# lzhangbj/DualVar

Measured on AMD Instinct MI355X. Metric: clips/sec (whole node), S3D-G 8x112^2 SimCLR pretrain step, higher is better.
Workload: dtype fp32

## Files before the change

dualvar_amd/csrc/conv.hip:

```cpp
#include "conv_common.hpp"

int dvt_conv_tap_kind(const void* conv_args, int mode);
int dvt_conv_tap_rows(const void* conv_args, int mode);
int dvt_conv_tap_launch(const void* conv_args, int mode, void* stream);
int64_t dvt_bn_ws_floats(int64_t rows, int np);
int dvt_conv_pp_rows(const void* conv_args, int mode);
int dvt_conv_pp_launch(const void* conv_args, int mode, void* stream);
void dvx_dgrad_bn_tail_launch(const void* conv_args, int is_f32, void* stream);

namespace {

constexpr int conv_waves_per_simd(int es, int gvb, int bm, int bn) {
  return (es == 4 && gvb == 16 && bm == 256) ? 3 : (es != 2 || gvb != 16) ? 1 : (bm * bn == 128 * 64) ? 6 : (bm == 128 && bn == 128) ? 3 : 1;
}

template <typename T, int MODE, int GVB, int BM, int BN, int WAVES_M, int WAVES_N, int GM, int NS = 2, bool SPLIT = false,
          bool WF = false, bool BNL = false>
__global__ __launch_bounds__(WAVES_M * WAVES_N * 64)
__attribute__((amdgpu_waves_per_eu(conv_waves_per_simd(sizeof(T), GVB, BM, BN)))) void conv_gemm_kernel(ConvArgs a) {
  static_assert(!SPLIT || sizeof(T) == 4, "the bf16 split is the fp32 mode's product");
  static_assert(!WF || (SPLIT && GVB == 16), "pre-split weights belong to the fp32 split kernels");
  static_assert(!BNL || (WF && GM == 1 && MODE == MODE_FWD), "BatchNorm on load: forward, uniform-tap gathers, pre-split weights");
  constexpr bool DMA = (GVB == 16);
  static_assert(GM == 0 || DMA, "uniform-tap gathers are DMA only");
// ... 1954 lines not shown
    p.BI = 64; p.BJ = (tmk == 3 ? 3 : d->kt) * bc;
    p.nti = (d->Cout + 63) / 64; p.ntj = (d->cin_pitch + bc - 1) / bc;
    const int krows = tmk == 3 ? 3 : 1;
    if (tmk == 4) {
      p.BJ = 224; p.ntj = 1;
      p.nchunks = d->N * d->To * d->Ho;
    } else if (tmk == 3) {
      p.nchunks = (M + 63) / 64;
    } else {
      const int pxs = 64 / d->To;
      p.nchunks = (int)(((int64_t)d->N * d->Hi * d->Wi + pxs - 1) / pxs);
    }
    int splits = std::max(1, ((tmk == 2 || tmk == 4) ? 512 : 768) / (p.nti * p.ntj * krows));
    splits = std::min(splits, std::max(1, p.nchunks / 8));
    const double slab_us = 8.0 * d->Cout * (double)J / 4e6;
    const int s_opt = (int)(std::sqrt(p.nchunks * 1.2 / slab_us) + 0.5);
    splits = std::max(1, std::min(splits, s_opt));
    p.chunks_per_split = (p.nchunks + splits - 1) / splits;
    p.splits = (p.nchunks + p.chunks_per_split - 1) / p.chunks_per_split;
    p.rows_per_split = p.chunks_per_split * 64;
    p.slab_stride = ((long long)d->Cout * J + 63) / 64 * 64;
    return p;
  }
  static const int f32s_force = env_int("DUALVAR_WGRAD_F32S", -1);
  const int f32s_pick = (f32s_force == 0 || f32s_force == 2) ? f32s_force : -1;
  if (p.dma && d->dtype == DV_F32 && !f32_exact() && f32s_pick >= 0) {
    p.f32s = f32s_pick;
    dvx_wgrad_f32s_tile(f32s_pick, &p.BI, &p.BJ);
    per_cu = std::max(1, std::min(2, 163840 / dvx_wgrad_f32s_lds_bytes(f32s_pick)));
  } else if (p.dma) {
    const WgradCfg* tab = d->dtype == DV_F32 ? kWgF32 : kWgBf16;
    const int ncfg = d->dtype == DV_F32 ? 2 : 4;
    constexpr int minrows_ = 256;
    double best = 0;
    for (int c = 0; c < ncfg; ++c) {
      const WgradCfg& k = tab[c];
      const int nti = (d->Cout + k.BI - 1) / k.BI, ntj = (J + k.BJ - 1) / k.BJ;
      const double fill = (double)M * nti * ntj * (k.BI + k.BJ) * es / 18e12;
      const double mfma = 2.0 * M * (double)(nti * k.BI) * (ntj * k.BJ) / (d->dtype == DV_F32 ? 120e12 : 1600e12);
      const int cap = 256 * wgrad_wgs_per_cu(es, k.BI, k.BJ, k.WVI * k.WVJ, k.NS);
      const int64_t sp = std::max<int64_t>(1, std::min<int64_t>(cap / (nti * ntj), (M + minrows_ - 1) / minrows_));
      const double wgs = (double)nti * ntj * sp;
      const double t = std::max(fill, mfma) * std::max(1.0, 256.0 / wgs);
      if (p.cfg < 0 || t < best) { best = t; p.cfg = c; }
    }
    const WgradCfg& k = tab[p.cfg];
    p.BI = k.BI; p.BJ = k.BJ;
    per_cu = wgrad_wgs_per_cu(es, k.BI, k.BJ, k.WVI * k.WVJ, k.NS);
  } else {
    const bool narrow = (d->Cout + 63) / 64 * 64 < (d->Cout + 127) / 128 * 128;
    p.BI = narrow ? 64 : 128;
    p.BJ = narrow ? 128 : 64;
  }
  p.nti = (d->Cout + p.BI - 1) / p.BI;
  p.ntj = (J + p.BJ - 1) / p.BJ;
  const int tiles = p.nti * p.ntj;
  constexpr int minrows = 256;
  const int tgt = 256 * per_cu;
  int splits = tgt / tiles;
  const int max_splits = (M + minrows - 1) / minrows;
  if (splits > max_splits) splits = max_splits;
  {
    const double t_step = d->dtype == DV_F32 ? 1.5 : 0.7;
    const double slab_us = 8.0 * d->Cout * (double)J / 4e6;
    const int s_opt = (int)(std::sqrt(M / 32.0 * t_step / slab_us) + 0.5);
    if (splits > s_opt) splits = s_opt;
  }
  if (splits < 1) splits = 1;
  p.rows_per_split = ((M + splits - 1) / splits + 31) / 32 * 32;
  p.splits = (M + p.rows_per_split - 1) / p.rows_per_split;
  p.slab_stride = ((long long)d->Cout * J + 63) / 64 * 64;
  return p;
}

extern "C" int dv_conv3d_wgrad_tile(const dv_conv_desc* d, int32_t* rows, int32_t* cols, int32_t* splits) {
  if (!d || !rows || !cols || !splits) return DV_EINVAL;
  int rc = check_desc(d);
  if (rc) return rc;
  const WgradPlan p = plan_wgrad(d);
  *rows = p.BI; *cols = p.BJ; *splits = p.splits;
  return DV_OK;
}

extern "C" int64_t dv_conv3d_wgrad_workspace(const dv_conv_desc* d) {
  if (check_desc(d)) return 0;
  const WgradPlan p = plan_wgrad(d);
  return p.splits > 1 ? (int64_t)p.splits * p.slab_stride * 4 : 0;
}

static bool wgrad_plan_is_share(const dv_conv_desc* d, const WgradPlan& p) {
  if (p.tm) return wgrad_tm_kind(d) == 4;
  return p.dma && d->dtype == DV_F32 && !f32_exact() && p.f32s < 0 && p.cfg == 1;
}
extern "C" int dv_conv3d_wgrad_bn_ok(const dv_conv_desc* d) {
  if (!d || check_desc(d)) return 0;
  return wgrad_plan_is_share(d, plan_wgrad(d)) ? 1 : 0;
}

static int wgrad_impl(const dv_conv_desc* d, const void* x, const void* dy, float* dw, void* workspace,
                      int64_t workspace_bytes, const dv_bn_bwd* bn, void* stream, const dv_bn_in* bn_in = nullptr) {
  int rc = check_desc(d);
  if (rc) return rc;
  if (!x || !dy || !dw) return DV_EINVAL;
  if (!aligned16(dy) || !aligned16(dw) || (reinterpret_cast<uintptr_t>(x) & 7)) return DV_EALIGN;
  const WgradPlan p = plan_wgrad(d);
  if (bn_in) {
    if (bn || !bn_in->scale || !bn_in->shift) return DV_EINVAL;
    const int k = p.tm ? wgrad_tm_kind(d) : 0;
    if (k != 1 && k != 2) return DV_EUNSUPPORTED;
  }
  if (bn) {
    if (!bn->x || !bn->mean || !bn->invstd || !bn->gamma || !bn->sums || bn->n_rep <= 0) return DV_EINVAL;
    if ((bn->dgamma == nullptr) != (bn->dbeta == nullptr)) return DV_EINVAL;
    if (!(bn->flags & DV_NO_RELU_MASK) && (!bn->scale || !bn->shift)) return DV_EINVAL;
    if (bn->ldx != d->ldy) return DV_EINVAL;
    if (!aligned16(bn->x)) return DV_EALIGN;
    if (!wgrad_plan_is_share(d, p)) return DV_EUNSUPPORTED;
  }
  const int64_t need = p.splits > 1 ? (int64_t)p.splits * p.slab_stride * 4 : 0;
  if (need && (!workspace || workspace_bytes < need)) return DV_EINVAL;
  if (need && !aligned16(workspace)) return DV_EALIGN;
  if (p.gvb == 16 && !aligned16(x)) return DV_EALIGN;
  WgradArgs a;
  fill_geom(d, MODE_FWD, a.g);
  a.x = x; a.dy = dy; a.dw = dw;
  a.slab = need ? reinterpret_cast<float*>(workspace) : nullptr;
  a.slab_stride = p.slab_stride;
  a.M = d->N * d->To * d->Ho * d->Wo;
  a.Cout = d->Cout; a.CoutP = d->cout_pitch; a.J = a.g.Ktot;
  a.ldx = d->ldx; a.ldy = d->ldy; a.ldw = a.g.Ktot;
  a.nti = p.nti; a.ntj = p.ntj;
  a.rows_per_split = p.rows_per_split;
  a.perm = make_row_perm(d->kt > 1 && d->To > 1, d->To, d->Ho * d->Wo);
  const int grid = p.nti * p.ntj * p.splits;
  const bool narrow = p.BI == 64;
  hipStream_t s = (hipStream_t)stream;
  if (p.tm) {
    TmWgradArgs t;
    t.x = x; t.dy = dy; t.dw = dw; t.slab = a.slab; t.slab_stride = p.slab_stride;
    t.S = d->Hi * d->Wi; t.NQ = d->N * t.S; t.T = d->To; t.kind = wgrad_tm_kind(d);
    t.Cout = d->Cout; t.CoutP = d->cout_pitch; t.CP = d->cin_pitch;
    t.ldx = d->ldx; t.ldy = d->ldy; t.ldw = a.ldw;
    t.nti = p.nti; t.ntc = p.ntj; t.nchunks = p.nchunks; t.chunks_per_split = p.chunks_per_split;
    t.x_bytes = (int)(((int64_t)d->N * d->Ti * d->Hi * d->Wi - 1) * d->ldx * 4 + (int64_t)d->cin_pitch * 4);
    t.dy_bytes = (int)(((int64_t)a.M - 1) * d->ldy * 4 + (int64_t)d->cout_pitch * 4);
    t.fS = make_fastdiv((uint32_t)t.S);
    t.M = a.M; t.H = d->Hi; t.W = d->Wi;
    t.fW = make_fastdiv((uint32_t)d->Wi); t.fH = make_fastdiv((uint32_t)d->Hi);
    t.Wo = d->Wo; t.Ho = d->Ho; t.Wp = d->Wi; t.Hp = d->Hi;
    t.bn_x = nullptr;
    if (bn_in) { t.in_scale = bn_in->scale; t.in_shift = bn_in->shift; t.in_C = d->Cin; t.in_relu = (bn_in->flags & DV_RELU) ? 1 : 0; }
    if (t.kind == 4) {
      t.fH = make_fastdiv((uint32_t)d->Ho);
      if (bn) {
        t.bn_x = bn->x; t.bn_mean = bn->mean; t.bn_invstd = bn->invstd; t.bn_gamma = bn->gamma; t.bn_scale = bn->scale;
        t.bn_shift = bn->shift; t.bn_sums = bn->sums; t.bn_dgamma = bn->dgamma; t.bn_dbeta = bn->dbeta;
        t.bn_inv_count = bn->inv_count; t.bn_dscale = bn->dparam_scale; t.bn_rep = bn->n_rep;
        t.bn_mask = (bn->flags & DV_NO_RELU_MASK) ? 0 : 1;
      }
    }
    dvw_wgrad_tm_launch(&t, t.kind == 3 ? grid * 3 : grid, stream);
  } else if (p.dma) {
    const int64_t es = d->dtype == DV_F32 ? 4 : 2;
    WgradDmaArgs aa;
    aa.w = a;
    aa.x_bytes = (int)(((int64_t)d->N * d->Ti * d->Hi * d->Wi - 1) * d->ldx * es + (int64_t)d->cin_pitch * es);
    aa.dy_bytes = (int)(((int64_t)a.M - 1) * d->ldy * es + (int64_t)d->cout_pitch * es);
    aa.bn_x = nullptr;
    if (bn) {
      aa.bn_x = bn->x; aa.bn_mean = bn->mean; aa.bn_invstd = bn->invstd; aa.bn_gamma = bn->gamma; aa.bn_scale = bn->scale;
      aa.bn_shift = bn->shift; aa.bn_sums = bn->sums; aa.bn_dgamma = bn->dgamma; aa.bn_dbeta = bn->dbeta;
      aa.bn_inv_count = bn->inv_count; aa.bn_dscale = bn->dparam_scale; aa.bn_rep = bn->n_rep;
      aa.bn_mask = (bn->flags & DV_NO_RELU_MASK) ? 0 : 1;
    }
#define WGD(T_, BI_, BJ_, WI_, WJ_, NS_, ...) \
  hipLaunchKernelGGL((conv_wgrad_dma_kernel<T_, BI_, BJ_, WI_, WJ_, NS_, ##__VA_ARGS__>), dim3(grid), dim3(WI_ * WJ_ * 64), 0, s, aa)
    if (p.f32s >= 0) {
      dvx_launch_wgrad_f32s(p.f32s, &aa, grid, s);
    } else if (d->dtype == DV_BF16) {
      switch (p.cfg) {
        case 0: WGD(bf16_t, 128, 128, 2, 2, 3); break;
        case 1: WGD(bf16_t, 64, 256, 1, 4, 3); break;
        case 2: WGD(bf16_t, 128, 256, 2, 2, 3); break;
        default: WGD(bf16_t, 192, 256, 3, 4, 4); break;
      }
    } else {
      if (f32_exact()) {
        if (p.cfg == 1) WGD(float, 64, 128, 2, 2, 2);
        else WGD(float, 128, 128, 2, 2, 2);
      } else {
        if (bn) WGD(float, 64, 128, 1, 4, 2, true, true, true);
        else if (p.cfg == 1) WGD(float, 64, 128, 1, 4, 2, true, true);
        else WGD(float, 128, 128, 2, 2, 2, true);
      }
    }
#undef WGD
  } else {
#define WG_LAUNCH(T_, G_)                                                                                   \
  do {                                                                                                      \
    if (narrow) hipLaunchKernelGGL((conv_wgrad_kernel<T_, G_, 64, 128>), dim3(grid), dim3(256), 0, s, a);   \
    else hipLaunchKernelGGL((conv_wgrad_kernel<T_, G_, 128, 64>), dim3(grid), dim3(256), 0, s, a);          \
  } while (0)
    if (d->dtype == DV_F32) WG_LAUNCH(float, 16);
    else if (p.gvb == 16) WG_LAUNCH(bf16_t, 16);
    else WG_LAUNCH(bf16_t, 8);
#undef WG_LAUNCH
  }
  if (need) {
    const long long n4 = (long long)d->Cout * a.ldw / 4;
    hipLaunchKernelGGL(wgrad_reduce_kernel, dim3((unsigned)((n4 + 15) / 16)), dim3(256), 0, s, a.slab, p.slab_stride,
                       p.splits, dw, n4);
  }
  return dv_launch_status();
}

extern "C" int dv_conv3d_wgrad(const dv_conv_desc* d, const void* x, const void* dy, float* dw, void* workspace,
                               int64_t workspace_bytes, void* stream) {
  return wgrad_impl(d, x, dy, dw, workspace, workspace_bytes, nullptr, stream);
}

extern "C" int dv_conv3d_wgrad_bn(const dv_conv_desc* d, const void* x, const void* g, float* dw, void* workspace,
                                  int64_t workspace_bytes, const dv_bn_bwd* bn, void* stream) {
  if (!bn) return DV_EINVAL;
  return wgrad_impl(d, x, g, dw, workspace, workspace_bytes, bn, stream);
}

extern "C" int dv_conv3d_wgrad_bn_in(const dv_conv_desc* d, const void* x_bn, const dv_bn_in* bn, const void* dy, float* dw,
                                     void* workspace, int64_t workspace_bytes, void* stream) {
  if (!bn) return DV_EINVAL;
  return wgrad_impl(d, x_bn, dy, dw, workspace, workspace_bytes, nullptr, stream, bn);
}

extern "C" int dv_conv3d_bn_in_ok(const dv_conv_desc* d) {
  if (!d || check_desc(d)) return 0;
  const int k = wgrad_tm_kind(d);
  if (k != 1 && k != 2) return 0;
  return fwd_bn_in_path(d);
}
```

dualvar_amd/csrc/conv_common.hpp:

```cpp
#pragma once
#include "common.hpp"
#include <algorithm>
#include <cmath>
#include <cstdlib>
#include <type_traits>
#include <utility>


namespace {


enum { MODE_FWD = 0, MODE_DGRAD = 1 };

struct ConvGeom {
  int rT, rH, rW;
  int sT, sH, sW;
  int kt, kh, kw;
  int st, sh, sw;
  int pt, ph, pw;
  int CP;
  int Ktot;
  FastDiv dW, dH, dT;
};

// ... 192 lines not shown
};
template <> struct Mma<fp8e5_t> {
  static __device__ __forceinline__ void tile(const unsigned char* a_row, const unsigned char* b_row, int h, int sa, int sb, f32x16& acc) {
    mma_fp8<1, 0>(a_row, b_row, h, sa, sb, acc);
  }
};
template <typename T> struct OutOf { typedef T type; };
template <> struct OutOf<fp8e4_t> { typedef bf16_t type; };
template <> struct OutOf<fp8e5_t> { typedef bf16_t type; };

struct Split3 { bf16x8 hi, mid, lo; };
__device__ __forceinline__ Split3 split3(const float (&v)[8]) {
  Split3 s;
#pragma unroll
  for (int e = 0; e < 8; ++e) {
    const bf16_t h = (bf16_t)v[e];
    const float r1 = v[e] - (float)h;
    const bf16_t m = (bf16_t)r1;
    const float r2 = r1 - (float)m;
    s.hi[e] = h; s.mid[e] = m; s.lo[e] = (bf16_t)r2;
  }
  return s;
}
__device__ __forceinline__ void split3w_pair(float x0, float x1, unsigned& H, unsigned& Mi, unsigned& Lo) {
  typedef __attribute__((ext_vector_type(2))) float f32x2;
  typedef __attribute__((ext_vector_type(2))) unsigned u32x2;
  typedef __attribute__((ext_vector_type(2))) __bf16 bf16x2;
  const u32x2 mask = {0xffff0000u, 0xffff0000u};
  const f32x2 x = {x0, x1};
  const bf16x2 hb = __builtin_convertvector(x, bf16x2);
  const unsigned hw = __builtin_bit_cast(unsigned, hb);
  const u32x2 hwide = {hw << 16, hw & 0xffff0000u};
  const f32x2 r1 = x - __builtin_bit_cast(f32x2, hwide);
  const u32x2 rb = __builtin_bit_cast(u32x2, r1);
  const f32x2 r2 = r1 - __builtin_bit_cast(f32x2, rb & mask);
  const u32x2 qb = __builtin_bit_cast(u32x2, r2);
  H = hw;
  Mi = __builtin_amdgcn_perm(rb.y, rb.x, 0x07060302u);
  Lo = __builtin_amdgcn_perm(qb.y, qb.x, 0x07060302u);
}
__device__ __forceinline__ Split3 split3w(const float (&v)[8]) {
  typedef __attribute__((ext_vector_type(4))) unsigned u32x4v;
  u32x4v H, Mi, Lo;
#pragma unroll
  for (int p = 0; p < 4; ++p) {
    unsigned h_, m_, l_;
    split3w_pair(v[2 * p], v[2 * p + 1], h_, m_, l_);
    H[p] = h_; Mi[p] = m_; Lo[p] = l_;
  }
  Split3 s;
  s.hi = __builtin_bit_cast(bf16x8, H); s.mid = __builtin_bit_cast(bf16x8, Mi); s.lo = __builtin_bit_cast(bf16x8, Lo);
  return s;
}
template <class F, int... Is>
__device__ __forceinline__ void static_for_impl(F&& f, std::integer_sequence<int, Is...>) { (f(std::integral_constant<int, Is>()), ...); }
template <int N, class F>
__device__ __forceinline__ void static_for(F&& f) { static_for_impl(f, std::make_integer_sequence<int, N>()); }
__device__ __forceinline__ void mma_split3(const Split3& a, const Split3& b, f32x16& acc) {
  acc = __builtin_amdgcn_mfma_f32_32x32x16_bf16(a.mid, b.mid, acc, 0, 0, 0);
  acc = __builtin_amdgcn_mfma_f32_32x32x16_bf16(a.hi, b.lo, acc, 0, 0, 0);
  acc = __builtin_amdgcn_mfma_f32_32x32x16_bf16(a.lo, b.hi, acc, 0, 0, 0);
  acc = __builtin_amdgcn_mfma_f32_32x32x16_bf16(a.hi, b.mid, acc, 0, 0, 0);
  acc = __builtin_amdgcn_mfma_f32_32x32x16_bf16(a.mid, b.hi, acc, 0, 0, 0);
  acc = __builtin_amdgcn_mfma_f32_32x32x16_bf16(a.hi, b.hi, acc, 0, 0, 0);
}
__device__ __forceinline__ Split3 split3_row(const unsigned char* row, int h, int s) {
  const f32x4 lo4 = *reinterpret_cast<const f32x4*>(row + ((2 * h) ^ s) * 16);
  const f32x4 hi4 = *reinterpret_cast<const f32x4*>(row + ((2 * h + 1) ^ s) * 16);
  const float v[8] = {lo4.x, lo4.y, lo4.z, lo4.w, hi4.x, hi4.y, hi4.z, hi4.w};
  return split3(v);
}

__device__ __forceinline__ float act_apply(float v, int flags) {
  if (flags & DV_RELU) v = fmaxf(v, 0.f);
  if (flags & DV_SIGMOID) v = 1.f / (1.f + __expf(-v));
  return v;
}

struct WgradArgs {
  const void* x;
  const void* dy;
  float* dw;
  float* slab;
  long long slab_stride;
  int M, Cout, CoutP, J;
  int ldx, ldy, ldw;
  int nti, ntj;
  int rows_per_split;
  ConvGeom g;
  RowPerm perm;
};

__device__ __forceinline__ void wgrad_store_block(const WgradArgs& a, int split, int row0, int col, int h, const f32x16& acc) {
  if (col >= a.J) return;
#pragma unroll
  for (int r = 0; r < 16; ++r) {
    const int row = row0 + (r & 3) + 8 * (r >> 2) + 4 * h;
    if (row < a.Cout) {
      const size_t e = (size_t)row * a.ldw + col;
      if (a.slab) a.slab[(size_t)split * a.slab_stride + e] = acc[r];
      else a.dw[e] += acc[r];
    }
  }
}


struct WgradDmaArgs {
  WgradArgs w;
  int x_bytes, dy_bytes;
  const void* bn_x;
  const float *bn_mean, *bn_invstd, *bn_gamma, *bn_scale, *bn_shift, *bn_sums;
  float *bn_dgamma, *bn_dbeta;
  float bn_inv_count, bn_dscale;
  int bn_rep, bn_mask;
};

template <int RB> __device__ __forceinline__ int wg_swz(int row) { return (RB % 256) ? ((row >> 1) & 1) : (row & 3); }

template <int RB>
__device__ __forceinline__ bf16x8 wg_frag(const unsigned char* tile, int col0, int lane, int ks) {
  const int g16 = lane >> 4, li = lane & 15;
  const int q = li >> 2, p = li & 3;
  const int row = ks * 16 + 8 * (g16 >> 1) + q;
  const int colb = ((col0 + 16 * (g16 & 1) + 4 * p) * 2) ^ (wg_swz<RB>(q) << 6);
  const unsigned char* ad = tile + row * RB + colb;
  s16x4 lo = __builtin_amdgcn_ds_read_tr16_b64_v4i16((__attribute__((address_space(3))) s16x4*)(ad));
  s16x4 hi = __builtin_amdgcn_ds_read_tr16_b64_v4i16((__attribute__((address_space(3))) s16x4*)(ad + 4 * RB));
  s16x8 v = {lo.x, lo.y, lo.z, lo.w, hi.x, hi.y, hi.z, hi.w};
  return __builtin_bit_cast(bf16x8, v);
}

struct TmWgradArgs {
  const void* x;
  const void* dy;
  float* dw;
  float* slab;
  long long slab_stride;
  int NQ, S, T;
  int Cout, CoutP, CP;
  int ldx, ldy, ldw;
  int nti, ntc;
  int nchunks, chunks_per_split;
  int x_bytes, dy_bytes;
  int kind;
  FastDiv fS;
  int M, H, W;
  FastDiv fW, fH;
  int Wo, Ho, Wp, Hp;
  const void* bn_x;
  const float *bn_mean, *bn_invstd, *bn_gamma, *bn_scale, *bn_shift, *bn_sums;
  float *bn_dgamma, *bn_dbeta;
  float bn_inv_count, bn_dscale;
  int bn_rep, bn_mask;
  const float* in_scale = nullptr;
  const float* in_shift = nullptr;
  int in_C = 0, in_relu = 0;
};

}
```

dualvar_amd/csrc/conv_tap_wgrad.hip:

```cpp
#include "conv_common.hpp"

namespace {

__device__ __forceinline__ void tw_gload16(f32x4& dst, dma_rsrc_t rsrc, unsigned voff) {
  asm volatile("buffer_load_dwordx4 %0, %1, %2, 0 offen" : "=v"(dst) : "v"(voff), "s"(rsrc) : "memory");
}
__device__ __forceinline__ void tw_gload16_hi(f32x4& dst, dma_rsrc_t rsrc, unsigned voff) {
  asm volatile("buffer_load_dwordx4 %0, %1, %2, 0 offen offset:16" : "=v"(dst) : "v"(voff), "s"(rsrc) : "memory");
}

__device__ __forceinline__ bf16x8 wg_frag64(const unsigned char* tile, int lane, int ks) {
  const int g16 = lane >> 4, li = lane & 15;
  const int q = li >> 2, p = li & 3;
  const int row = ks * 16 + 8 * (g16 >> 1) + q;
  const unsigned char* ad = tile + row * 64 + (16 * (g16 & 1) + 4 * p) * 2;
  s16x4 lo = __builtin_amdgcn_ds_read_tr16_b64_v4i16((__attribute__((address_space(3))) s16x4*)(ad));
  s16x4 hi = __builtin_amdgcn_ds_read_tr16_b64_v4i16((__attribute__((address_space(3))) s16x4*)(ad + 4 * 64));
  s16x8 v = {lo.x, lo.y, lo.z, lo.w, hi.x, hi.y, hi.z, hi.w};
  return __builtin_bit_cast(bf16x8, v);
}

template <int YT, int XT, int KT, int ST, int PT, int BC, bool BNL = false>
__global__ __launch_bounds__(256) __attribute__((amdgpu_waves_per_eu(BC == 64 ? 3 : 2, BC == 64 ? 3 : 2))) void conv_wgrad_tm_kernel(TmWgradArgs a) {
  constexpr int PXS = 64 / YT, KS = PXS / 16, YROWS = 64, XROWS = XT * PXS;
// ... 208 lines not shown
  f32x4 sreg[4][2];
  auto issue = [&](int chunk) {
    const int r0 = chunk * R;
#pragma unroll
    for (int k = 0; k < 4; ++k) {
      const int u = (tid + 256 * k) & 511;
      const int grow = k >= 2 ? r0 + xshift + 2 + (u >> 3) : r0 + (u >> 3);
      const bool ok = grow >= 0 && grow < a.M && ucolb[k] != kOOB;
      const unsigned off = ok ? (unsigned)grow * (k >= 2 ? ldxb : ldyb) + ucolb[k] : kOOB;
      tw_gload16(sreg[k][0], k >= 2 ? x_rs : dy_rs, off);
      tw_gload16_hi(sreg[k][1], k >= 2 ? x_rs : dy_rs, off);
    }
  };
  auto split_unit = [&](const f32x4 (&r)[2]) -> Split3 {
    const float v[8] = {r[0].x, r[0].y, r[0].z, r[0].w, r[1].x, r[1].y, r[1].z, r[1].w};
    return split3w(v);
  };
  auto write_unit = [&](unsigned off, int plane, const Split3& q3) {
    *reinterpret_cast<bf16x8*>(smem + off) = q3.hi;
    *reinterpret_cast<bf16x8*>(smem + off + plane) = q3.mid;
    *reinterpret_cast<bf16x8*>(smem + off + 2 * plane) = q3.lo;
  };

  f32x16 acc[3];
#pragma unroll
  for (int d = 0; d < 3; ++d)
#pragma unroll
    for (int r = 0; r < 16; ++r) acc[d][r] = 0.f;

  if (tid < 8) *reinterpret_cast<f32x4*>(smem + ZOFF + tid * 16) = f32x4{0.f, 0.f, 0.f, 0.f};
  if (ch_begin < ch_end && tid < 16) {
    const int prow = tid >> 3, ch8 = tid & 7;
    const int grow = ch_begin * R + xshift + prow, cbase = c0 + ch8 * 8;
    const bool ok = grow >= 0 && grow < a.M && cbase + 8 <= a.CP;
    f32x4 t2[2];
    const unsigned off = ok ? (unsigned)grow * ldxb + (unsigned)cbase * 4u : kOOB;
    tw_gload16(t2[0], x_rs, off);
    tw_gload16_hi(t2[1], x_rs, off);
    asm volatile("s_waitcnt vmcnt(0)" : "+v"(t2[0]), "+v"(t2[1])::"memory");
    write_unit((unsigned)(YOP + prow * RB + ((ch8 ^ (wg_swz<RB>(prow) << 2)) << 4)), XPLANE, split_unit(t2));
  }
  const int g16 = lane >> 4, li = lane & 15, fq = li >> 2, fp = li & 3;
  const int frow = 8 * (g16 >> 1) + fq;
  const unsigned fcol = (unsigned)((bj * 32 + 16 * (g16 & 1) + 4 * fp) * 2);
  const unsigned zaddr = (unsigned)ZOFF + fcol % RB;

  if (ch_begin < ch_end) issue(ch_begin);
  for (int ch = ch_begin; ch < ch_end; ++ch) {
    asm volatile("s_waitcnt vmcnt(0)"
                 : "+v"(sreg[0][0]), "+v"(sreg[0][1]), "+v"(sreg[1][0]), "+v"(sreg[1][1]), "+v"(sreg[2][0]), "+v"(sreg[2][1]),
                   "+v"(sreg[3][0]), "+v"(sreg[3][1])::"memory");
    Split3 sp[2];
#pragma unroll
    for (int k = 0; k < 2; ++k) sp[k] = split_unit(sreg[k]);
    bf16x8 carry = {};
    const bool carrier = ch > ch_begin && tid < 48;
    const unsigned csrc = (unsigned)(YOP + (tid >> 4) * XPLANE + (64 + ((tid >> 3) & 1)) * RB + (tid & 7) * 16);
    if (carrier) carry = *reinterpret_cast<const bf16x8*>(smem + csrc);
    unsigned long long inv0 = 0, inv1 = 0, inv2 = 0;
    if (wave == 0) {
      const int m = ch * R + lane;
      uint32_t q_, ww, hh, q2;
      fd_divmod((uint32_t)m, a.fW, q_, ww);
      fd_divmod(q_, a.fH, q2, hh);
      const bool bad_h = (unsigned)((int)hh + dh - 1) >= (unsigned)a.H || m >= a.M;
      inv0 = __ballot(bad_h || ww == 0);
      inv1 = __ballot(bad_h);
      inv2 = __ballot(bad_h || (int)ww == a.W - 1);
    }
    __syncthreads();
    if (carrier) *reinterpret_cast<bf16x8*>(smem + csrc - 64 * RB) = carry;
#pragma unroll
    for (int k = 0; k < 2; ++k) write_unit(uwr[k], YPLANE, sp[k]);
#pragma unroll
    for (int k = 2; k < 4; ++k) write_unit(uwr[k], XPLANE, split_unit(sreg[k]));
    if (wave == 0 && lane == 0) {
      unsigned* mw = reinterpret_cast<unsigned*>(smem + MOFF);
      mw[0] = (unsigned)inv0; mw[1] = (unsigned)(inv0 >> 32); mw[2] = (unsigned)inv1; mw[3] = (unsigned)(inv1 >> 32);
      mw[4] = (unsigned)inv2; mw[5] = (unsigned)(inv2 >> 32);
    }
    __syncthreads();
    if (ch + 1 < ch_end) issue(ch + 1);
    const unsigned* mw = reinterpret_cast<const unsigned*>(smem + MOFF);
#pragma unroll
    for (int ks = 0; ks < KS; ++ks) {
      Split3 av;
      av.hi = wg_frag<RB>(smem, bi * 32, lane, ks);
      av.mid = wg_frag<RB>(smem + YPLANE, bi * 32, lane, ks);
      av.lo = wg_frag<RB>(smem + 2 * YPLANE, bi * 32, lane, ks);
#pragma unroll
      for (int dw = 0; dw < 3; ++dw) {
        const unsigned mword = mw[dw * 2 + (ks >> 1)];
        const int r_lo = (ks & 1) * 16 + frow;
        const int xr = ks * 16 + frow + dw;
        const unsigned a_lo = (unsigned)(YOP + xr * RB) + (fcol ^ ((unsigned)wg_swz<RB>(xr) << 6));
        const unsigned ad_lo = ((mword >> r_lo) & 1u) ? zaddr : a_lo;
        const unsigned ad_hi = ((mword >> (r_lo + 4)) & 1u) ? zaddr : a_lo + 4 * RB;
        Split3 b;
        {
          auto rd = [&](unsigned lo_, unsigned hi_) -> bf16x8 {
            s16x4 lo = __builtin_amdgcn_ds_read_tr16_b64_v4i16((__attribute__((address_space(3))) s16x4*)(smem + lo_));
            s16x4 hi = __builtin_amdgcn_ds_read_tr16_b64_v4i16((__attribute__((address_space(3))) s16x4*)(smem + hi_));
            s16x8 v = {lo.x, lo.y, lo.z, lo.w, hi.x, hi.y, hi.z, hi.w};
            return __builtin_bit_cast(bf16x8, v);
          };
          const unsigned p1l = ad_lo == zaddr ? 0u : (unsigned)XPLANE, p1h = ad_hi == zaddr ? 0u : (unsigned)XPLANE;
          b.hi = rd(ad_lo, ad_hi);
          b.mid = rd(ad_lo + p1l, ad_hi + p1h);
          b.lo = rd(ad_lo + 2 * p1l, ad_hi + 2 * p1h);
        }
        mma_split3(av, b, acc[dw]);
      }
    }
  }

  const int nrow0 = i0 + bi * 32, cc = c0 + bj * 32 + l31;
  if (cc < a.CP) {
#pragma unroll
    for (int dw = 0; dw < 3; ++dw) {
#pragma unroll
      for (int r = 0; r < 16; ++r) {
        const int n = nrow0 + (r & 3) + 8 * (r >> 2) + 4 * h;
        if (n < a.Cout) {
          const size_t e = (size_t)n * a.ldw + (size_t)(dh * 3 + dw) * a.CP + cc;
          if (a.slab) a.slab[(size_t)split * a.slab_stride + e] = acc[dw][r];
          else a.dw[e] += acc[dw][r];
        }
      }
    }
  }
}

template <bool BNA>
__global__ __launch_bounds__(256) __attribute__((amdgpu_waves_per_eu(2, 2))) void conv_wgrad_pp_kernel(TmWgradArgs a) {
  constexpr int KH = 7, KS = 4, RBY = 128, XROWS = 68, XRB = 16;
  constexpr int YPLANE = 64 * RBY, YOP = 3 * YPLANE;
  constexpr int XLINE = XROWS * XRB, XPLANE = KH * XLINE, XOP = 3 * XPLANE;
  constexpr int COFF = YOP + XOP;
  constexpr unsigned kOOB = 0x80000000u;
  __shared__ __attribute__((aligned(1024))) unsigned char smem[COFF + 5 * 64 * 4];
  const int tid = threadIdx.x, lane = tid & 63;
  const int wave = __builtin_amdgcn_readfirstlane(tid >> 6);
  const int h = lane >> 5, l31 = lane & 31;
  int bid = xcd_remap((int)blockIdx.x, (int)gridDim.x);
  const int tile_i = bid % a.nti;
  const int split = bid / a.nti;
  const int i0 = tile_i * 64;
  const int bi = wave >> 1, par = wave & 1;
  const int ln_begin = split * a.chunks_per_split, ln_end = min(a.nchunks, ln_begin + a.chunks_per_split);
  const dma_rsrc_t x_rs = dma_make_rsrc(a.x, (unsigned)a.x_bytes), dy_rs = dma_make_rsrc(a.dy, (unsigned)a.dy_bytes);
  const dma_rsrc_t bx_rs = dma_make_rsrc(BNA ? a.bn_x : a.dy, (unsigned)a.dy_bytes);
  const unsigned ldyb = (unsigned)a.ldy * 4u;
  const int Wo = a.Wo, Wp = a.Wp;

  for (int o = tid * 16; o < COFF; o += 256 * 16) *reinterpret_cast<f32x4*>(smem + o) = f32x4{0.f, 0.f, 0.f, 0.f};
  if constexpr (BNA) {
    if (tid < 64) {
      const int c = i0 + tid, cpb = (a.Cout + 7) & ~7;
      float k1 = 0.f, k2 = 0.f, k3 = 0.f, sc = 0.f, sh = 0.f;
      if (c < a.Cout) {
        float sg = 0.f, sgx = 0.f;
        for (int r = 0; r < a.bn_rep; ++r) { sg += a.bn_sums[(size_t)r * 2 * cpb + c]; sgx += a.bn_sums[(size_t)r * 2 * cpb + cpb + c]; }
        k1 = a.bn_gamma[c] * a.bn_invstd[c];
        k2 = -k1 * a.bn_invstd[c] * sgx * a.bn_inv_count;
        k3 = -k1 * sg * a.bn_inv_count - k2 * a.bn_mean[c];
        if (a.bn_mask) { sc = a.bn_scale[c]; sh = a.bn_shift[c]; }
        if (split == 0 && a.bn_dgamma) {
          a.bn_dbeta[c] += a.bn_dscale * sg;
          a.bn_dgamma[c] += a.bn_dscale * sgx;
        }
      }
      float* cf = reinterpret_cast<float*>(smem + COFF);
      cf[tid] = k1; cf[64 + tid] = k2; cf[128 + tid] = k3; cf[192 + tid] = sc; cf[256 + tid] = sh;
    }
  }

  const int ch8 = tid & 7;
  const unsigned ycol = i0 + ch8 * 8 + 8 <= a.CoutP ? (unsigned)(i0 + ch8 * 8) * 4u : kOOB;
  unsigned ywr[2], xwr[2], xsrc[2];
  bool yok[2], xok[2];
#pragma unroll
  for (int k = 0; k < 2; ++k) {
    const int u = tid + 256 * k, row = u >> 3;
    yok[k] = row < Wo && ycol != kOOB;
    ywr[k] = (unsigned)(row * RBY + ((ch8 ^ (wg_swz<RBY>(row) << 2)) << 4));
    const int dh = u / Wp, wp = u - dh * Wp;
    xok[k] = u < KH * Wp;
    xwr[k] = (unsigned)(YOP + dh * XLINE + wp * XRB);
    xsrc[k] = (unsigned)((dh * Wp + wp) * 32);
  }
  f32x4 greg[2][2], breg[2][2], xreg[2][2];
  auto issue = [&](int line) {
    const unsigned m0 = (unsigned)line * (unsigned)Wo;
    const unsigned img = fd_div((uint32_t)line, a.fH);
    const unsigned ho = (unsigned)line - img * (unsigned)a.Ho;
    const unsigned xline0 = ((img * (unsigned)a.Hp + 2u * ho) * (unsigned)Wp) * 32u;
#pragma unroll
    for (int k = 0; k < 2; ++k) {
      const unsigned yo = yok[k] ? (m0 + (unsigned)((tid + 256 * k) >> 3)) * ldyb + ycol : kOOB;
      tw_gload16(greg[k][0], dy_rs, yo);
      tw_gload16_hi(greg[k][1], dy_rs, yo);
      if constexpr (BNA) {
        tw_gload16(breg[k][0], bx_rs, yo);
        tw_gload16_hi(breg[k][1], bx_rs, yo);
      }
      const unsigned xo = xok[k] ? xline0 + xsrc[k] : kOOB;
      tw_gload16(xreg[k][0], x_rs, xo);
      tw_gload16_hi(xreg[k][1], x_rs, xo);
    }
  };
  auto write3 = [&](unsigned off, int plane, const Split3& q3) {
    *reinterpret_cast<bf16x8*>(smem + off) = q3.hi;
    *reinterpret_cast<bf16x8*>(smem + off + plane) = q3.mid;
    *reinterpret_cast<bf16x8*>(smem + off + 2 * plane) = q3.lo;
  };

  f32x16 acc[4];
#pragma unroll
  for (int d = 0; d < 4; ++d)
#pragma unroll
    for (int r = 0; r < 16; ++r) acc[d][r] = 0.f;

  const int g16 = lane >> 4, li = lane & 15, fq = li >> 2, fp = li & 3;
  const int cg = (g16 & 1) * 4 + fp;
  const unsigned xlane = (unsigned)(YOP + (8 * (g16 >> 1) + fq + (cg >> 1)) * XRB + (cg & 1) * 8);

  __syncthreads();
  if (ln_begin < ln_end) issue(ln_begin);
  for (int ln = ln_begin; ln < ln_end; ++ln) {
    if constexpr (BNA)
      asm volatile("s_waitcnt vmcnt(0)"
                   : "+v"(greg[0][0]), "+v"(greg[0][1]), "+v"(greg[1][0]), "+v"(greg[1][1]), "+v"(breg[0][0]), "+v"(breg[0][1]),
                     "+v"(breg[1][0]), "+v"(breg[1][1]), "+v"(xreg[0][0]), "+v"(xreg[0][1]), "+v"(xreg[1][0]), "+v"(xreg[1][1])::"memory");
    else
      asm volatile("s_waitcnt vmcnt(0)"
                   : "+v"(greg[0][0]), "+v"(greg[0][1]), "+v"(greg[1][0]), "+v"(greg[1][1]), "+v"(xreg[0][0]), "+v"(xreg[0][1]),
                     "+v"(xreg[1][0]), "+v"(xreg[1][1])::"memory");
    Split3 sy[2];
#pragma unroll
    for (int k = 0; k < 2; ++k) {
      float v[8] = {greg[k][0].x, greg[k][0].y, greg[k][0].z, greg[k][0].w, greg[k][1].x, greg[k][1].y, greg[k][1].z, greg[k][1].w};
      if constexpr (BNA) {
        const float xv[8] = {breg[k][0].x, breg[k][0].y, breg[k][0].z, breg[k][0].w, breg[k][1].x, breg[k][1].y, breg[k][1].z, breg[k][1].w};
        const float* cf = reinterpret_cast<const float*>(smem + COFF) + ch8 * 8;
#pragma unroll
        for (int e = 0; e < 8; ++e) {
          const float act = xv[e] * cf[192 + e] + cf[256 + e];
          const float gg = (a.bn_mask && !(act > 0.f)) ? 0.f : v[e];
          v[e] = cf[e] * gg + cf[64 + e] * xv[e] + cf[128 + e];
        }
      }
      sy[k] = split3w(v);
    }
    __syncthreads();
#pragma unroll
    for (int k = 0; k < 2; ++k) {
      if (yok[k]) write3(ywr[k], YPLANE, sy[k]);
      if (xok[k]) {
        const float v[8] = {xreg[k][0].x, xreg[k][0].y, xreg[k][0].z, xreg[k][0].w, xreg[k][1].x, xreg[k][1].y, xreg[k][1].z, xreg[k][1].w};
        write3(xwr[k], XPLANE, split3w(v));
      }
    }
    __syncthreads();
    if (ln + 1 < ln_end) issue(ln + 1);
#pragma unroll
    for (int ks = 0; ks < KS; ++ks) {
      Split3 av;
      av.hi = wg_frag<RBY>(smem, bi * 32, lane, ks);
      av.mid = wg_frag<RBY>(smem + YPLANE, bi * 32, lane, ks);
      av.lo = wg_frag<RBY>(smem + 2 * YPLANE, bi * 32, lane, ks);
#pragma unroll
      for (int d = 0; d < 4; ++d) {
        const int dh = 2 * d + par;
        if (dh >= KH) continue;
        const unsigned ad = xlane + (unsigned)(dh * XLINE + ks * 16 * XRB);
        auto rd = [&](unsigned o) -> bf16x8 {
          s16x4 lo = __builtin_amdgcn_ds_read_tr16_b64_v4i16((__attribute__((address_space(3))) s16x4*)(smem + o));
          s16x4 hi = __builtin_amdgcn_ds_read_tr16_b64_v4i16((__attribute__((address_space(3))) s16x4*)(smem + o + 4 * XRB));
          s16x8 v = {lo.x, lo.y, lo.z, lo.w, hi.x, hi.y, hi.z, hi.w};
          return __builtin_bit_cast(bf16x8, v);
        };
        Split3 b;
        b.hi = rd(ad); b.mid = rd(ad + XPLANE); b.lo = rd(ad + 2 * XPLANE);
        mma_split3(av, b, acc[d]);
      }
    }
  }

  const int nrow0 = i0 + bi * 32;
#pragma unroll
  for (int d = 0; d < 4; ++d) {
    const int dh = 2 * d + par;
    if (dh >= KH) continue;
#pragma unroll
    for (int r = 0; r < 16; ++r) {
      const int n = nrow0 + (r & 3) + 8 * (r >> 2) + 4 * h;
      if (n < a.Cout) {
        const size_t e = (size_t)n * a.ldw + (size_t)dh * 32 + l31;
        if (a.slab) a.slab[(size_t)split * a.slab_stride + e] = acc[d][r];
        else a.dw[e] += acc[d][r];
      }
    }
  }
}

}

void dvw_wgrad_tm_launch(const void* args, int grid, void* stream) {
  const TmWgradArgs& a = *static_cast<const TmWgradArgs*>(args);
  hipStream_t s = (hipStream_t)stream;
  if (a.kind == 4) {
    if (a.bn_x) hipLaunchKernelGGL((conv_wgrad_pp_kernel<true>), dim3(grid), dim3(256), 0, s, a);
    else hipLaunchKernelGGL((conv_wgrad_pp_kernel<false>), dim3(grid), dim3(256), 0, s, a);
  } else if (a.kind == 3) hipLaunchKernelGGL((conv_wgrad_sp_kernel<0>), dim3(grid), dim3(256), 0, s, a);
  else if (a.in_scale != nullptr) {
    if (a.kind == 2) hipLaunchKernelGGL((conv_wgrad_tm_kernel<4, 8, 7, 2, 3, 32, true>), dim3(grid), dim3(256), 0, s, a);
    else if (a.T == 4) hipLaunchKernelGGL((conv_wgrad_tm_kernel<4, 4, 3, 1, 1, 64, true>), dim3(grid), dim3(256), 0, s, a);
    else hipLaunchKernelGGL((conv_wgrad_tm_kernel<2, 2, 3, 1, 1, 64, true>), dim3(grid), dim3(256), 0, s, a);
  }
  else if (a.kind == 2) hipLaunchKernelGGL((conv_wgrad_tm_kernel<4, 8, 7, 2, 3, 32>), dim3(grid), dim3(256), 0, s, a);
  else if (a.T == 4) hipLaunchKernelGGL((conv_wgrad_tm_kernel<4, 4, 3, 1, 1, 64>), dim3(grid), dim3(256), 0, s, a);
  else hipLaunchKernelGGL((conv_wgrad_tm_kernel<2, 2, 3, 1, 1, 64>), dim3(grid), dim3(256), 0, s, a);
}
```

Measured before the change: 7958.

## Reuse input rows across output lines in the wgrad kernel via an LDS ring

In the tap-major wgrad kernel (kind 4), consecutive output lines of the same image share most of their KH input rows. The x tile in LDS is now a ring buffer indexed by a rotating base, and on carried lines only the two new input rows are loaded and split instead of all KH rows. This is meant to cut global loads and bf16 split work for the x operand. It adds modular slot arithmetic to the LDS read addresses, and an env var can restore the old full restaging.

```diff
diff --git a/dualvar_amd/csrc/conv.hip b/dualvar_amd/csrc/conv.hip
--- a/dualvar_amd/csrc/conv.hip
+++ b/dualvar_amd/csrc/conv.hip
@@ -2130,6 +2130,7 @@
     if (bn_in) { t.in_scale = bn_in->scale; t.in_shift = bn_in->shift; t.in_C = d->Cin; t.in_relu = (bn_in->flags & DV_RELU) ? 1 : 0; }
     if (t.kind == 4) {
       t.fH = make_fastdiv((uint32_t)d->Ho);
+      t.pp_restage = env_int("DUALVAR_WGRAD_PP_RESTAGE", 0) ? 1 : 0;
       if (bn) {
         t.bn_x = bn->x; t.bn_mean = bn->mean; t.bn_invstd = bn->invstd; t.bn_gamma = bn->gamma; t.bn_scale = bn->scale;
         t.bn_shift = bn->shift; t.bn_sums = bn->sums; t.bn_dgamma = bn->dgamma; t.bn_dbeta = bn->dbeta;
diff --git a/dualvar_amd/csrc/conv_common.hpp b/dualvar_amd/csrc/conv_common.hpp
--- a/dualvar_amd/csrc/conv_common.hpp
+++ b/dualvar_amd/csrc/conv_common.hpp
@@ -368,6 +368,7 @@
   float *bn_dgamma, *bn_dbeta;
   float bn_inv_count, bn_dscale;
   int bn_rep, bn_mask;
+  int pp_restage = 0;
   const float* in_scale = nullptr;
   const float* in_shift = nullptr;
   int in_C = 0, in_relu = 0;
diff --git a/dualvar_amd/csrc/conv_tap_wgrad.hip b/dualvar_amd/csrc/conv_tap_wgrad.hip
--- a/dualvar_amd/csrc/conv_tap_wgrad.hip
+++ b/dualvar_amd/csrc/conv_tap_wgrad.hip
@@ -384,6 +384,10 @@
   const dma_rsrc_t bx_rs = dma_make_rsrc(BNA ? a.bn_x : a.dy, (unsigned)a.dy_bytes);
   const unsigned ldyb = (unsigned)a.ldy * 4u;
   const int Wo = a.Wo, Wp = a.Wp;
+  const bool ring = !a.pp_restage;
+  auto carried = [&](int line) -> bool {
+    return ring && line != ln_begin && (unsigned)line != fd_div((uint32_t)line, a.fH) * (unsigned)a.Ho;
+  };
 
   for (int o = tid * 16; o < COFF; o += 256 * 16) *reinterpret_cast<f32x4*>(smem + o) = f32x4{0.f, 0.f, 0.f, 0.f};
   if constexpr (BNA) {
@@ -421,8 +425,11 @@
     xwr[k] = (unsigned)(YOP + dh * XLINE + wp * XRB);
     xsrc[k] = (unsigned)((dh * Wp + wp) * 32);
   }
+  const bool cok = tid < 2 * Wp;
+  const int cdh = tid >= Wp ? 1 : 0, cwp = tid - cdh * Wp;
+  const unsigned csrc = (unsigned)((5 * Wp + tid) * 32);
   f32x4 greg[2][2], breg[2][2], xreg[2][2];
-  auto issue = [&](int line) {
+  auto issue = [&](int line, bool carry) {
     const unsigned m0 = (unsigned)line * (unsigned)Wo;
     const unsigned img = fd_div((uint32_t)line, a.fH);
     const unsigned ho = (unsigned)line - img * (unsigned)a.Ho;
@@ -436,9 +443,15 @@
         tw_gload16(breg[k][0], bx_rs, yo);
         tw_gload16_hi(breg[k][1], bx_rs, yo);
       }
-      const unsigned xo = xok[k] ? xline0 + xsrc[k] : kOOB;
-      tw_gload16(xreg[k][0], x_rs, xo);
-      tw_gload16_hi(xreg[k][1], x_rs, xo);
+      if (!carry) {
+        const unsigned xo = xok[k] ? xline0 + xsrc[k] : kOOB;
+        tw_gload16(xreg[k][0], x_rs, xo);
+        tw_gload16_hi(xreg[k][1], x_rs, xo);
+      } else if (k == 0) {
+        const unsigned xo = cok ? xline0 + csrc : kOOB;
+        tw_gload16(xreg[0][0], x_rs, xo);
+        tw_gload16_hi(xreg[0][1], x_rs, xo);
+      }
     }
   };
   auto write3 = [&](unsigned off, int plane, const Split3& q3) {
@@ -458,8 +471,11 @@
   const unsigned xlane = (unsigned)(YOP + (8 * (g16 >> 1) + fq + (cg >> 1)) * XRB + (cg & 1) * 8);
 
   __syncthreads();
-  if (ln_begin < ln_end) issue(ln_begin);
+  if (ln_begin < ln_end) issue(ln_begin, false);
+  int base = 0;
   for (int ln = ln_begin; ln < ln_end; ++ln) {
+    const bool carry = carried(ln);
+    base = carry ? (base + 2 >= KH ? base + 2 - KH : base + 2) : 0;
     if constexpr (BNA)
       asm volatile("s_waitcnt vmcnt(0)"
                    : "+v"(greg[0][0]), "+v"(greg[0][1]), "+v"(greg[1][0]), "+v"(greg[1][1]), "+v"(breg[0][0]), "+v"(breg[0][1]),
@@ -488,13 +504,15 @@
 #pragma unroll
     for (int k = 0; k < 2; ++k) {
       if (yok[k]) write3(ywr[k], YPLANE, sy[k]);
-      if (xok[k]) {
+      if (carry ? (k == 0 && cok) : xok[k]) {
         const float v[8] = {xreg[k][0].x, xreg[k][0].y, xreg[k][0].z, xreg[k][0].w, xreg[k][1].x, xreg[k][1].y, xreg[k][1].z, xreg[k][1].w};
-        write3(xwr[k], XPLANE, split3w(v));
-      }
-    }
-    __syncthreads();
-    if (ln + 1 < ln_end) issue(ln + 1);
+        int slot = base + 5 + cdh;
+        slot = slot >= KH ? slot - KH : slot;
+        write3(carry ? (unsigned)(YOP + slot * XLINE + cwp * XRB) : xwr[k], XPLANE, split3w(v));
+      }
+    }
+    __syncthreads();
+    if (ln + 1 < ln_end) issue(ln + 1, carried(ln + 1));
 #pragma unroll
     for (int ks = 0; ks < KS; ++ks) {
       Split3 av;
@@ -505,7 +523,8 @@
       for (int d = 0; d < 4; ++d) {
         const int dh = 2 * d + par;
         if (dh >= KH) continue;
-        const unsigned ad = xlane + (unsigned)(dh * XLINE + ks * 16 * XRB);
+        const int slot = base + dh >= KH ? base + dh - KH : base + dh;
+        const unsigned ad = xlane + (unsigned)(slot * XLINE + ks * 16 * XRB);
         auto rd = [&](unsigned o) -> bf16x8 {
           s16x4 lo = __builtin_amdgcn_ds_read_tr16_b64_v4i16((__attribute__((address_space(3))) s16x4*)(smem + o));
           s16x4 hi = __builtin_amdgcn_ds_read_tr16_b64_v4i16((__attribute__((address_space(3))) s16x4*)(smem + o + 4 * XRB));
```

Result: no change. 7957 (median of 6 runs) (-0.0%).
